# instaclustr/atsc

Hardware: AMD Instinct MI355X
Metric: Msamples/sec compressed (auto, e=5%) (higher is better)
Workload: dtype f64; 1 GPU; BASELINE.json configs[2] per GPU: 10,485,760 f64 samples, 40960 frames x 256, --compressor auto, e=5% (max_error=(float)5/100), classes C0-C4 cycled per 65536-sample block, inputs resident in HBM; the timed loop rotates over 5 different resident batches (series ids 0..4, batch b with the block -> class mapping shifted by 2 b); frames_per_gpu=40960, frame_len=256, encoded_bytes_rank0=3592754, parallelism=single GPU, GPU_MAX_HW_QUEUES=4

## Files before the change

atsc_amd/csrc/atsc_device.h:

```cpp
#pragma once
#include <hip/hip_runtime.h>
#include <stdint.h>

#include "../../include/atsc_hip.h"
#include "atsc_internal.h"

#include <map>
#include <mutex>
#include <utility>

namespace atsc {

#define DEVI __device__ __forceinline__
template <int W = 0>
DEVI uint32_t tid_now()
{
    uint32_t t = (W == 1) ? __builtin_amdgcn_mbcnt_hi(~0u, __builtin_amdgcn_mbcnt_lo(~0u, 0u)) : threadIdx.x;
    asm volatile("" : "+v"(t));
    return t;
}

inline hipError_t ensure_dyn_lds(const void *fn, uint32_t bytes)
{
    static std::mutex mu;
// ... 158 lines not shown
    v += dpp_u32<0x111, 0xf>(v);
    v += dpp_u32<0x112, 0xf>(v);
    v += dpp_u32<0x114, 0xf>(v);
    v += dpp_u32<0x118, 0xf>(v);
    v += dpp_u32<0x142, 0xa>(v);
    v += dpp_u32<0x143, 0xc>(v);
    return v;
}
DEVI uint32_t wave_max_u32(uint32_t v)
{
    v = max(v, dpp_u32<0xb1, 0xf>(v));
    v = max(v, dpp_u32<0x4e, 0xf>(v));
    v = max(v, dpp_u32<0x124, 0xf>(v));
    v = max(v, dpp_u32<0x128, 0xf>(v));
    v = max(v, dpp_u32<0x142, 0xa>(v));
    v = max(v, dpp_u32<0x143, 0xc>(v));
    return (uint32_t)__builtin_amdgcn_readlane((int)v, 63);
}
DEVI uint32_t wave_min_u32(uint32_t v) { return ~wave_max_u32(~v); }
template <int CTRL, int ROWMASK>
DEVI double dpp_f64(double v)
{
    const int lo = __builtin_amdgcn_update_dpp(0, __double2loint(v), CTRL, ROWMASK, 0xf, false);
    const int hi = __builtin_amdgcn_update_dpp(0, __double2hiint(v), CTRL, ROWMASK, 0xf, false);
    return __hiloint2double(hi, lo);
}
template <int CTRL>
DEVI double dpp_f64_full(double v)
{
    const int lo = __builtin_amdgcn_mov_dpp(__double2loint(v), CTRL, 0xf, 0xf, true);
    const int hi = __builtin_amdgcn_mov_dpp(__double2hiint(v), CTRL, 0xf, 0xf, true);
    return __hiloint2double(hi, lo);
}
DEVI double wave_sum_f64(double v)
{
    v += dpp_f64_full<0xb1>(v);
    v += dpp_f64_full<0x4e>(v);
    v += dpp_f64_full<0x124>(v);
    v += dpp_f64_full<0x128>(v);
    v += dpp_f64<0x142, 0xa>(v);
    v += dpp_f64<0x143, 0xc>(v);
    const int lo = __builtin_amdgcn_readlane(__double2loint(v), 63);
    const int hi = __builtin_amdgcn_readlane(__double2hiint(v), 63);
    return __hiloint2double(hi, lo);
}

template <int FN, int T, int MAXIT = 0, typename F>
DEVI void for_strided(uint32_t tid, uint32_t n, F &&f)
{
    if constexpr (FN != 0) {
#pragma unroll
        for (int m = 0; m < (FN + T - 1) / T; ++m) {
            const uint32_t j = tid + (uint32_t)(m * T);
            if (FN % T == 0 || j < (uint32_t)FN) f(j);
        }
    } else if constexpr (MAXIT != 0) {
#pragma unroll
        for (int m = 0; m < MAXIT; ++m) {
            const uint32_t j = tid + (uint32_t)(m * T);
            if (j < n) f(j);
        }
    } else {
        for (uint32_t j = tid; j < n; j += T) f(j);
    }
}

template <int W>
DEVI double block_sum_f64(double v, double *red, int &parity)
{
    v = wave_sum_f64(v);
    if (W == 1) return v;
    double *r = red + parity * 16;
    parity ^= 1;
    if ((tid_now<W>() & 63) == 0) r[tid_now<W>() >> 6] = v;
    __syncthreads();
    double s = r[0];
#pragma unroll
    for (int w = 1; w < W; ++w) s += r[w];
    return s;
}
template <int W>
DEVI uint32_t block_sum_u32(uint32_t v, double *red, int &parity)
{
    v = wave_sum_u32(v);
    if (W == 1) return v;
    uint32_t *r = (uint32_t *)(red + parity * 16);
    parity ^= 1;
    if ((tid_now<W>() & 63) == 0) r[tid_now<W>() >> 6] = v;
    __syncthreads();
    uint32_t s = r[0];
#pragma unroll
    for (int w = 1; w < W; ++w) s += r[w];
    return s;
}

template <int CTRL, int ROWMASK>
DEVI double dpp_f64_self(double v)
{
    const int lo = __builtin_amdgcn_update_dpp(__double2loint(v), __double2loint(v), CTRL, ROWMASK, 0xf, false);
    const int hi = __builtin_amdgcn_update_dpp(__double2hiint(v), __double2hiint(v), CTRL, ROWMASK, 0xf, false);
    return __hiloint2double(hi, lo);
}
template <bool IsMin>
DEVI double wave_minmax_f64(double v)
{
#define ATSC_MM_STEP(O)                                          \
    {                                                            \
        const double o = O;                                      \
        v = IsMin ? fmin(o, v) : fmax(o, v);                     \
    }
    ATSC_MM_STEP(dpp_f64_full<0xb1>(v))
    ATSC_MM_STEP(dpp_f64_full<0x4e>(v))
    ATSC_MM_STEP(dpp_f64_full<0x124>(v))
    ATSC_MM_STEP(dpp_f64_full<0x128>(v))
    ATSC_MM_STEP((dpp_f64_self<0x142, 0xa>(v)))
    ATSC_MM_STEP((dpp_f64_self<0x143, 0xc>(v)))
// ... 227 lines not shown
    return X;
}

template <typename KnotFn>
DEVI double spline_eval(KnotFn V, uint32_t i, uint32_t n, uint32_t step, uint32_t K, uint32_t magic)
{
    if (i == n - 1) return V(K - 1);
    uint32_t seg = (step == 1) ? i : __umulhi(i, magic);
    if (seg > K - 2) seg = K - 2;
    const uint32_t t0i = seg * step;
    const uint32_t t1i = (seg + 1 == K - 1) ? (n - 1) : (seg + 1) * step;
    const double t0 = (double)t0i, t1 = (double)t1i;
    const double v0 = V(seg), v1 = V(seg + 1);
    const double nt = ((double)i - t0) / (t1 - t0);
    if (seg > 0 && K - seg > 2) {
        const uint32_t tmi = (seg - 1) * step;
        const uint32_t tpi = (seg + 2 == K - 1) ? (n - 1) : (seg + 2) * step;
        const double tm = (double)tmi, tp = (double)tpi;
        const double vm = V(seg - 1), vp = V(seg + 2);
        const double t2 = nt * nt;
        const double t3 = t2 * nt;
        const double two_t3 = t3 * 2.0;
        const double two_t2 = t2 * 2.0;
        const double three_t2 = t2 * 3.0;
        const double m0 = (v1 - vm) / (t1 - tm) * (t1 - t0);
        const double m1 = (vp - v0) / (tp - t0) * (t1 - t0);
        return v0 * (two_t3 - three_t2 + 1.0) + m0 * (t3 - two_t2 + nt) + v1 * (three_t2 - two_t3) +
               m1 * (t3 - t2);
    }
    return v0 * (1.0 - nt) + v1 * nt;
}

DEVI double div1e5(double r)
{
    const double y = 1.0e-5;
    const double q = r * y;
    const double rem = fma(-q, 100000.0, r);
    return fma(rem, y, q);
}
DEVI bool wide_range(double mn, double mx) { return !(fabs(mn) < 1e150 && fabs(mx) < 1e150); }
DEVI double div1e5_fix(double r, double o, bool wide) { return (wide && isinf(r)) ? r : o; }

DEVI double recip_abs(double g)
{
    const double a = fabs(g);
    if (a > 1e-290 && a < 1e290) {
        double r = __builtin_amdgcn_rcp(a);
        r = fma(fma(-a, r, 1.0), r, r);
        r = fma(fma(-a, r, 1.0), r, r);
        return r;
    }
    return 1.0 / a;
}
DEVI double mape_term(double o, double g)
{
    const double a = fabs(g), d = fabs(o - g);
    return (a > 1e-290 && a < 1e290) ? d * recip_abs(g) : d / a;
}
DEVI bool tiny_range(double mn, double mx) { return !(mn > 1e-290 || mx < -1e-290); }
DEVI double spline_term_slow(double sv, double mn, double mx, double g)
{
    double o = round(sv * 100000.0) / 100000.0;
    if (o < mn) o = mn;
    else if (o > mx) o = mx;
    return fabs((o - g) / g);
}
DEVI double fft_term_slow(float v, double mn, double mx, double g)
{
    double o = round((double)v * 100000.0) / 100000.0;
    if (o > mx) o = mx;
    if (o < mn) o = mn;
    return fabs((o - g) / g);
}

DEVI float hp_norm(uint64_t e) { return __uint_as_float((uint32_t)(e >> 32)); }
DEVI void hp_sift_down_range(uint64_t *h, uint32_t pos, uint32_t end)
{
    const uint64_t elt = h[pos];
    const float en = hp_norm(elt);
    uint32_t child = 2 * pos + 1;
    while (end >= 2 && child <= end - 2) {
        const uint64_t c0 = h[child], c1 = h[child + 1];
        const bool right = !(hp_norm(c0) > hp_norm(c1));
        const uint64_t c = right ? c1 : c0;
        child += right ? 1u : 0u;
        if (en >= hp_norm(c)) { h[pos] = elt; return; }
        h[pos] = c;
        pos = child;
        child = 2 * pos + 1;
    }
    if (end >= 1 && child == end - 1) {
        const uint64_t c = h[child];
        if (!(en >= hp_norm(c))) { h[pos] = c; pos = child; }
    }
    h[pos] = elt;
}
DEVI void hp_rebuild(uint64_t *h, uint32_t len)
{
    for (uint32_t n = len / 2; n > 0;) {
        --n;
        hp_sift_down_range(h, n, len);
    }
}
DEVI void hp_rebuild_parallel(uint64_t *h, uint32_t len, uint32_t tid, uint32_t nthreads)
{
    if (len < 2) return;
// ... 235 lines not shown
```

atsc_amd/csrc/atsc_host.cpp:

```cpp
#include <hip/hip_runtime.h>

#include <algorithm>
#include <chrono>
#include <cmath>
#include <cstdio>
#include <cstdlib>
#include <cstring>
#include <limits>
#include <map>
#include <memory>
#include <mutex>
#include <new>
#include <thread>
#include <string>
#include <vector>

#include "atsc_host_private.h"

namespace atsc {
hipError_t launch_compress_class(int cls, uint32_t count, uint32_t lds, const double *samples,
                                 const DevFrame *frames, const uint32_t *ids, const DevPlan *plans,
                                 const float2 *twpool, const KParams &prm, uint8_t *slots,
                                 DevResult *res, atsc_frame_diag *diag, const UniArgs &uni, hipStream_t s,
                                 hipEvent_t ev0 = nullptr, hipEvent_t ev1 = nullptr);
// ... 612 lines not shown
        } else {
            pi = it->second;
        }
        const DevPlan &dp = p->tabs.plans[pi];
        const int c = class_of(n, dp.L);
        if (c < 0) { atsc_plan_destroy(p); return fail(ctx, ATSC_E_UNSUPPORTED, "plan_create: frame class"); }
        cls[f] = c;
        p->class_count[c]++;
        p->class_lds[c] = std::max(p->class_lds[c], dp.lds_bytes);
        if (c == CLASS_LARGE) p->ws_stride = std::max(p->ws_stride, large_ws_bytes(n, dp.L, dp.kcap));
        frames[f].sample_off = frame_off[f];
        frames[f].slot_off = slot;
        frames[f].n = n;
        frames[f].plan = pi;
        const uint64_t pb = atsc_payload_bound_bytes(n);
        slot += (pb + 15) & ~15ull;
        bound += pb + 16;
    }
    p->n_samples = frame_off[n_frames] - frame_off[0];
    p->h_frames = frames;
    p->slot_bytes = slot;
    p->body_bound = bound;
    std::vector<uint32_t> ids(n_frames);
    {
        uint32_t acc = 0;
        for (int c = 0; c < N_CLASSES; ++c) { p->class_first[c] = acc; acc += p->class_count[c]; }
        std::vector<uint32_t> cur(p->class_first);
        for (uint64_t f = 0; f < n_frames; ++f) ids[cur[cls[f]]++] = (uint32_t)f;
    }
    p->class_uni.assign(N_CLASSES, UniArgs());
    for (int c = 0; c < N_CLASSES; ++c) {
        UniArgs &u = p->class_uni[c];
        memset(&u, 0, sizeof(u));
        const uint32_t cnt = p->class_count[c];
        if (!cnt) continue;
        const uint32_t *cid = ids.data() + p->class_first[c];
        const DevFrame &f0 = frames[cid[0]];
        const uint64_t stride = (atsc_payload_bound_bytes(f0.n) + 15) & ~15ull;
        bool ok = true;
        for (uint32_t i = 0; i < cnt && ok; ++i) {
            const DevFrame &f = frames[cid[i]];
            ok = cid[i] == cid[0] + i && f.plan == f0.plan &&
                 f.sample_off == f0.sample_off + (uint64_t)i * f0.n &&
                 f.slot_off == f0.slot_off + (uint64_t)i * stride;
        }
        if (ok && c != CLASS_LARGE && !getenv("ATSC_NO_UNIFORM")) {
            u.enabled = 1;
            u.fid0 = cid[0];
            u.sample_off0 = f0.sample_off;
            u.slot_off0 = f0.slot_off;
            u.slot_stride = stride;
            u.n = f0.n;
            u.plan = f0.plan;
        }
    }
    p->large_tiled = choose_large_tiled(p->class_count[CLASS_LARGE]);
    if (p->class_count[CLASS_LARGE]) {
        std::vector<uint32_t> lp;
        for (uint64_t f = 0; f < n_frames; ++f)
            if (cls[f] == CLASS_LARGE) lp.push_back(frames[f].plan);
        std::sort(lp.begin(), lp.end());
        lp.erase(std::unique(lp.begin(), lp.end()), lp.end());
        p->large_pre = large_pre_extents(p->tabs.plans, lp);
        p->large_pre.even_off = 1;
        for (uint64_t f = 0; f < n_frames; ++f)
            if (cls[f] == CLASS_LARGE && (frames[f].sample_off & 1ull)) p->large_pre.even_off = 0;
    }
    int rc = upload_tables(ctx, p->tabs);
    if (rc) { atsc_plan_destroy(p); return rc; }
    const uint32_t nb = (uint32_t)((n_frames + 1023) / 1024);
#define PCHK(call)                                                                     \
    do {                                                                               \
        hipError_t e__ = (call);                                                       \
        if (e__ != hipSuccess) { atsc_plan_destroy(p); return fail(ctx, ATSC_E_HIP, #call, e__); } \
    } while (0)
    PCHK(pool_alloc(ctx, (void **)&p->d_frames, n_frames * sizeof(DevFrame)));
    PCHK(hipMemcpy(p->d_frames, frames.data(), n_frames * sizeof(DevFrame), hipMemcpyHostToDevice));
    PCHK(pool_alloc(ctx, (void **)&p->d_ids, n_frames * sizeof(uint32_t)));
    PCHK(hipMemcpy(p->d_ids, ids.data(), n_frames * sizeof(uint32_t), hipMemcpyHostToDevice));
    PCHK(pool_alloc(ctx, (void **)&p->d_res, n_frames * sizeof(DevResult)));
    p->slots_bytes = std::max<uint64_t>(slot, 16);
    PCHK(pool_alloc(ctx, (void **)&p->d_slots, p->slots_bytes));
    PCHK(pool_alloc(ctx, (void **)&p->d_local, n_frames * sizeof(uint32_t)));
    PCHK(pool_alloc(ctx, (void **)&p->d_blocksum, (nb + 1) * sizeof(uint64_t)));
    if (p->class_count[CLASS_LARGE]) {
        p->ws_slots = (std::min<uint32_t>(p->class_count[CLASS_LARGE], large_ws_slots(p->ws_stride)) + 3u) & ~3u;
        PCHK(pool_alloc(ctx, (void **)&p->d_ws, p->ws_stride * p->ws_slots));
    }
#undef PCHK
    *out = p;
    return ATSC_OK;
    ATSC_API_END
}
extern "C" uint64_t atsc_plan_n_frames(const atsc_plan *p) { return p ? p->n_frames : 0; }
extern "C" uint64_t atsc_plan_n_samples(const atsc_plan *p) { return p ? p->n_samples : 0; }
extern "C" uint64_t atsc_plan_body_bound(const atsc_plan *p) { return p ? p->body_bound : 0; }

static const uint32_t COMPRESSION_SPEED[7] = {0x7fffffffu, 4096, 2048, 1024, 512, 256, 128};

static int build_sub(atsc_ctx *ctx, const atsc_plan *plan, uint32_t min_n, uint32_t force_n, bool nopad,
                     bool want_res, SubPlan **out)
{
    *out = nullptr;
    SubPlan *t = new (std::nothrow) SubPlan();
    if (!t) return ATSC_E_NOMEM;
    t->min_n = min_n;
// ... 312 lines not shown
            int rc = build_sub(ctx, plan, 0, 0, true, false, &t);
            if (rc) return rc;
            plan->nopad = t;
        }
        int rc = launch_sub(ctx, plan, plan->nopad, d_samples, prm, S.d_slots, S.d_res, d_diag, s, ws_set);
        if (rc) return rc;
        return pack();
    }
    int dominant = 0, last_c = 0;
    if (adapt) { prm.cost = CH.d_cost; want_order = true; }
    for (int c = 1; c < N_CLASSES; ++c)
        if (plan->class_count[c] > plan->class_count[dominant]) dominant = c;
    for (int c = 0; c < N_CLASSES; ++c)
        if (plan->class_count[c]) last_c = c;
    for (int c = 0; c < N_CLASSES; ++c) {
        if (!plan->class_count[c]) continue;
        const bool timed = ctx->profiling && c == dominant;
        const bool bracket = timed && c == CLASS_LARGE;
        hipEvent_t ev0 = nullptr, ev1 = nullptr;
        if (timed) {
            if (ctx->ev_used == ctx->ev_pool.size()) {
                hipEvent_t a, b;
                HIPCHK(ctx, hipEventCreateWithFlags(&a, hipEventReleaseToDevice));
                HIPCHK(ctx, hipEventCreateWithFlags(&b, hipEventReleaseToDevice));
                ctx->ev_pool.emplace_back(a, b);
            }
            ev0 = ctx->ev_pool[ctx->ev_used].first;
            ev1 = ctx->ev_pool[ctx->ev_used].second;
            if (bracket) HIPCHK(ctx, hipEventRecord(ev0, s));
        }
        if (pipelined && c == last_c && c != CLASS_LARGE && !ev1) {
            ev1 = CH.ev_codec;
            codec_attached = true;
        }
        hipError_t e;
        if (c == CLASS_LARGE) {
            KParams lp = prm;
            lp.large_tiled = plan->large_tiled ? 1u : 0u;
            const bool pre = plan->large_pre.tiles1 && (compressor == ATSC_AUTO || compressor == ATSC_FFT);
            e = launch_compress_large(plan->class_count[c], d_samples, plan->d_frames, plan->d_ids + plan->class_first[c],
                                      plan->tabs.d_plans, plan->tabs.d_tw, lp, S.d_slots, S.d_res, d_diag, ws_set,
                                      plan->ws_stride, plan->ws_slots, s, pre ? &plan->large_pre : nullptr);
        }
        else {
            UniArgs u = plan->class_uni[c];
            u.adaptive = (ids_main != plan->d_ids) ? 1u : 0u;
            u.count = plan->class_count[c];
            u.spread = 0;
            if (u.enabled && !u.adaptive && u.count >= 4096) {
                uint32_t sp = (uint32_t)((double)u.count * 0.6180339887) | 1u;
                auto gcd = [](uint32_t a, uint32_t b) { while (b) { const uint32_t t = a % b; a = b; b = t; } return a; };
                while (gcd(sp, u.count) != 1) sp += 2;
                u.spread = sp % u.count;
            }
            e = launch_compress_class(c, plan->class_count[c], plan->class_lds[c], d_samples,
                                      plan->d_frames, ids_main + plan->class_first[c],
                                      plan->tabs.d_plans, plan->tabs.d_tw, prm, S.d_slots,
                                      S.d_res, d_diag, u, s, ev0, ev1);
        }
        if (e != hipSuccess) return fail(ctx, ATSC_E_HIP, "launch k_compress", e);
        if (bracket) HIPCHK(ctx, hipEventRecord(ev1, s));
        if (timed) ctx->ev_used++;
    }
    return pack();
}

extern "C" int atsc_compress_plan_dev(atsc_ctx *ctx, const atsc_plan *plan, const double *d_samples,
                                      int compressor, int bounded, float max_error, int sample_level,
                                      uint8_t *d_body, uint64_t body_cap, uint64_t *d_rec_off,
                                      uint8_t *d_chosen, double *d_err, void *stream)
{
    ATSC_API_BEGIN
    return compress_impl(ctx, plan, d_samples, compressor, bounded, max_error, sample_level, d_body,
                         body_cap, d_rec_off, d_chosen, d_err, stream, false);
    ATSC_API_END
}
extern "C" int atsc_compress_plan_dev_pipelined(atsc_ctx *ctx, const atsc_plan *plan,
                                                const double *d_samples, int compressor, int bounded,
                                                float max_error, int sample_level, uint8_t *d_body,
                                                uint64_t body_cap, uint64_t *d_rec_off,
                                                uint8_t *d_chosen, double *d_err, void *stream)
{
    ATSC_API_BEGIN
    return compress_impl(ctx, plan, d_samples, compressor, bounded, max_error, sample_level, d_body,
                         body_cap, d_rec_off, d_chosen, d_err, stream, true);
    ATSC_API_END
}
extern "C" int atsc_ctx_set_adaptive_order(atsc_ctx *ctx, int on)
{
    if (!ctx) return ATSC_E_INVALID;
    ctx->adaptive_order = on != 0;
    return ATSC_OK;
}
extern "C" int atsc_plan_join(atsc_ctx *ctx, const atsc_plan *plan, void *stream)
{
    if (!ctx || !plan) return fail(ctx, ATSC_E_INVALID, "plan_join: null argument");
    for (int i = 0; i < 8; ++i)
        if (plan->chains[i].pending) HIPCHK(ctx, hipStreamWaitEvent((hipStream_t)stream, plan->chains[i].ev_done, 0));
    return ATSC_OK;
}
extern "C" int atsc_plan_input_release(atsc_ctx *ctx, const atsc_plan *plan, void *stream)
{
    if (!ctx || !plan) return fail(ctx, ATSC_E_INVALID, "plan_input_release: null argument");
    for (int i = 0; i < 8; ++i)
        if (plan->chains[i].pending) HIPCHK(ctx, hipStreamWaitEvent((hipStream_t)stream, plan->chains[i].ev_codec, 0));
    return ATSC_OK;
// ... 849 lines not shown
```

atsc_amd/csrc/atsc_internal.h:

```cpp
#pragma once
#include <stdint.h>
#include <new>
#include <stdexcept>
#include <vector>

namespace atsc {

struct DevPlan {
    uint32_t n;
    uint32_t L;
    uint32_t pre;
    uint32_t bins;
    uint32_t mf;
    uint32_t dk1;
    uint32_t dk2;
    uint32_t kcap;
    uint32_t direct;
    uint32_t half;
    uint32_t M;
    uint32_t sc;
    uint32_t nstages;
    uint32_t radix[14];
    uint32_t stmagic[14];
    uint32_t p2bins;
// ... 46 lines not shown
    uint64_t slot_off;
    uint32_t n;
    uint32_t plan;
};

struct DevResult {
    double err;
    uint32_t len;
    uint32_t chosen;
};

struct KParams {
    double max_err;
    double poly_target;
    double poly_q_hi;
    double poly_q_lo;
    int32_t max_err_m;
    int32_t mode;
    int32_t bounded;
    int32_t want_diag;
    int32_t debug_stop;
    int32_t trial;
    uint32_t trial_min_n;
    const DevResult *trial_res;
    uint32_t *cost;
    uint32_t large_tiled;
    uint32_t sparse_inv;
    uint32_t prestats;
    uint32_t tile_stats;
    uint32_t fast_skip;
    uint32_t prefft;
};
struct LargePre {
    uint32_t tiles1, tiles2, chunks;
    uint32_t m1_max, m2_max;
    uint32_t sp_tiles;
    uint32_t chunks_n;
    uint32_t cols243;
    uint32_t rows9p;
    uint32_t even_off;
};
constexpr uint32_t LARGE_SPLIT_MAX = 128;

struct UniArgs {
    uint32_t enabled;
    uint32_t adaptive;
    uint32_t fid0;
    uint64_t sample_off0;
    uint64_t slot_off0;
    uint64_t slot_stride;
    uint32_t n;
    uint32_t plan;
    uint32_t spread, count;
};

struct DevDFrame {
    uint64_t payload_off;
    uint64_t out_off;
    uint32_t payload_len;
    uint32_t n;
    uint32_t tag;
    uint32_t plan;
};

struct DevWTask {
    uint64_t dst;
    uint32_t frame;
    uint32_t lo, hi;
    uint32_t pad;
};
struct DevWGather {
    uint64_t src, dst;
    uint32_t len, pad;
};

constexpr uint32_t AGG_TILE = 2048;
struct DevAggPart {
    double sum, mn, mx;
    uint64_t count;
};
enum : uint32_t { AGG_FIRST = 1, AGG_LAST = 2 };
struct DevAggTile {
    uint64_t src, dst;
    uint32_t lo, hi;
    uint32_t win, flags;
};
struct DevAggComb {
    uint64_t head, tail, mid, dst;
    uint32_t n, g, win, final_;
};

struct DevMomPart {
    double mx, m2x, mt, m2t, c;
    uint64_t n;
};
struct DevPosTile {
    uint64_t src, dst, t0;
    uint32_t lo, hi;
};

struct DevDltPart {
    double up, down, after_falls, max_rise, max_fall;
    uint64_t pairs, rises, falls;
};
enum : uint32_t { DLT_CONT = 1, DLT_CARRY = 2 };
struct DevDltTile {
    uint64_t src, dst;
// ... 146 lines not shown
```

atsc_amd/csrc/atsc_kernels.hip:

```cpp
#include <hip/hip_runtime.h>
#include <hip/hip_ext.h>
#include <stdint.h>
#include <stdlib.h>
#include <algorithm>
#include <string.h>

#include "atsc_device.h"

namespace atsc {

template <int W>
DEVI void fft_untangle(const DevPlan &P, const float2 *Z, float2 *out, const float2 *tw)
{
    constexpr int T = 64 * W;
    const uint32_t M = P.M;
    for (uint32_t k = tid_now<W>(); k <= M; k += T) {
        const float2 zk = Z[k == M ? 0 : k];
        const float2 zm = Z[k == 0 ? 0 : M - k];
        const float2 a = make_float2(zk.x + zm.x, zk.y - zm.y);
        const float2 b = make_float2(zk.x - zm.x, zk.y + zm.y);
        const float2 t = cmul_conj_tw(make_float2(b.y, -b.x), tw[k]);
        out[k] = make_float2(0.5f * a.x + 0.5f * t.x, 0.5f * a.y + 0.5f * t.y);
    }
    __syncthreads();
// ... 210 lines not shown
        const uint32_t ra = rec[i];
        const uint64_t ka = (uint64_t)__double_as_longlong(xs[ra & 0xffffu]);
        uint32_t r = 0;
        for (uint32_t j = q; j < count; j += p) {
            const uint32_t rb = rec[j];
            const uint64_t kb = (uint64_t)__double_as_longlong(xs[rb & 0xffffu]);
            r += (kb < ka || (kb == ka && rb < ra)) ? 1u : 0u;
        }
        if (p == 1) rank[i] = r;
        else if (r) atomicAdd(&rank[i], r);
    }
    __syncthreads();
    for (uint32_t i = tid; i < count; i += T) tmp[rank[i]] = rec[i];
    __syncthreads();
    for (uint32_t i = tid; i < count; i += T) rec[i] = tmp[i];
    __syncthreads();
}

#ifdef ATSC_STAMPS
__device__ unsigned long long g_phase_cyc[64 * 16];
__device__ unsigned long long g_frame_span[4 * 65536 * 3];
#define PH(i) do { if (FN != 0) { const long long now_ = clock64(); \
    if (tid == 0) atomicAdd(&ph_acc[i], (unsigned long long)(now_ - ph_t)); ph_t = clock64(); } } while (0)
#else
#define PH(i) do {} while (0)
#endif
template <int W, int SPL, bool IDW, int FN, bool LEAN_ = (FN != 0)>
__device__ __forceinline__ void compress_frame(
    const double *__restrict__ samples, const DevFrame *__restrict__ frames,
    const uint32_t *__restrict__ ids, const DevPlan *__restrict__ plans,
    const float2 *__restrict__ twpool, const KParams &prm, uint8_t *__restrict__ slots,
    DevResult *__restrict__ res, atsc_frame_diag *__restrict__ diag, const UniArgs &uni, const uint32_t bid)
{
    constexpr int T = 64 * W;
    constexpr bool FIX_ = FN != 0;
    extern __shared__ __attribute__((aligned(16))) unsigned char smem[];
    const uint32_t tid = tid_now<W>();
    uint32_t fid;
    DevFrame fr;
    const long long t_start = prm.cost ? clock64() : 0;
#ifdef ATSC_STAMPS
    __shared__ unsigned long long ph_acc[16];
    if (tid < 16) ph_acc[tid] = 0;
    __syncthreads();
    long long ph_t = clock64();
    const uint32_t span0 = 3u * 65536u * (((uint32_t)prm.debug_stop >> 24) & 3u);
    if (FN != 0 && tid == 0 && bid < 65536) {
        g_frame_span[span0 + 3 * bid] = wall_clock64();
        g_frame_span[span0 + 3 * bid + 2] = (unsigned long long)__builtin_amdgcn_s_getreg((31 << 11) | (0 << 6) | 4) |
                                           ((unsigned long long)__builtin_amdgcn_s_getreg((31 << 11) | (0 << 6) | 20) << 32);
    }
#endif
    if (FIX_ || uni.enabled) {
        const uint32_t r = uni.adaptive ? (uint32_t)__builtin_amdgcn_readfirstlane((int)(ids[bid] - uni.fid0))
                           : uni.spread ? (uint32_t)(((uint64_t)bid * uni.spread) % uni.count) : bid;
        fid = uni.fid0 + r;
        fr.sample_off = uni.sample_off0 + (uint64_t)r * uni.n;
        fr.slot_off = uni.slot_off0 + (uint64_t)r * uni.slot_stride;
        fr.n = uni.n;
        fr.plan = uni.plan;
    } else {
        fid = ids[bid];
        fr = frames[fid];
    }
    typedef const __attribute__((address_space(4))) DevPlan PlanConst;
    PlanConst &P = *(PlanConst *)(plans + fr.plan);
#define P_GENERIC (*(const DevPlan *)&P)
    constexpr bool FIX = FN != 0;
    constexpr bool LEAN = LEAN_;
    static_assert(LEAN || !FIX, "fixed-length instantiations are lean");
    constexpr uint32_t cL = FIX ? cx_next_size(FIX ? FN : 1) : 0, cmf = (3 >= FN / 100) ? 3 : FN / 100;
    static_assert(!FIX || (FN >= 128 && cL <= 64 * W * SPL), "fixed-length instantiation");
    constexpr bool chalf = cL % 2 == 0;
    constexpr uint32_t cM = chalf ? cL / 2 : cL;
    const uint32_t n = FIX ? FN : P.n, L = FIX ? cL : P.L, pre = FIX ? (cL - FN) / 2 : P.pre;
    const uint32_t bins = FIX ? cL / 2 + 1 : P.bins;
    const uint32_t mf = FIX ? cmf : P.mf;
    constexpr uint32_t cdk1 = cmf / 2 > 1 ? cmf / 2 : 1, cdk2 = cmf / 10 > 1 ? cmf / 10 : 1;
    constexpr uint32_t ckcap = (cL / 2 + 1 < cmf + 17 * cdk1 + 5 * cdk2) ? cL / 2 + 1 : cmf + 17 * cdk1 + 5 * cdk2;
    const uint32_t dk1 = FIX ? cdk1 : P.dk1, dk2 = FIX ? cdk2 : P.dk2;
    constexpr EncLds lay = enc_lds(FIX ? FN : 1, FIX ? cL : 1, FIX ? cM : 1, false, ckcap, W == 1);
    const uint32_t o_xs = FIX ? lay.o_xs : P.o_xs, o_tw = FIX ? lay.o_tw : P.o_tw, o_ab = FIX ? lay.o_ab : P.o_ab;
    const uint32_t ab_half = FIX ? lay.ab_half : P.ab_half, ab_bytes = FIX ? lay.ab_bytes : P.ab_bytes;
    const uint32_t o_sel = FIX ? lay.o_sel : P.o_sel, o_aux = FIX ? lay.o_aux : P.o_aux, o_red = FIX ? lay.o_red : P.o_red;
    const uint32_t o_hist = FIX ? lay.o_hist : P.o_hist;
    const uint32_t kcap = FIX ? ckcap : P.kcap;

    double *xs = (double *)(smem + o_xs);
    float2 *tw = (float2 *)(smem + o_tw);
    unsigned char *AB = smem + o_ab;
    float2 *A = (float2 *)AB;
    float2 *B = (float2 *)(AB + ab_half);
    Sel *sel = (Sel *)(smem + o_sel);
    uint32_t *aux = (uint32_t *)(smem + o_aux);
    double *red = (double *)(smem + o_red);
    uint32_t *wsum = (W == 1) ? (uint32_t *)red : (uint32_t *)(red + 32);
    int parity = 0;

    uint8_t *out = slots + fr.slot_off;
    int mode = LEAN ? (int)ATSC_AUTO : prm.mode;
    const bool bounded = LEAN ? true : (prm.bounded != 0);

    constexpr bool REGSTAT = FIX && W == 1 && (FN == 256 || FN == 512);
    bool reg_stats = false;
    double rs_mn = 0.0, rs_mx = 0.0;
    uint32_t rs_frac = 0, rs_pk = 0;
    {
        const double *src = samples + fr.sample_off;
        if constexpr (REGSTAT) {
            if ((fr.sample_off & 1ull) == 0) {
                constexpr int NP = FN / 128;
                const double2 *src2 = (const double2 *)src;
                double2 *xs2 = (double2 *)xs;
                double2 v[NP];
#pragma unroll
                for (int m = 0; m < NP; ++m) v[m] = src2[tid + 64 * m];
#pragma unroll
                for (int m = 0; m < NP; ++m) xs2[tid + 64 * m] = v[m];
                const double x0 = lane_f64(v[0].x, 0);
                rs_mn = x0;
                rs_mx = x0;
#pragma unroll
                for (int m = 0; m < NP; ++m) {
                    const double a = v[m].x, b = v[m].y;
                    rs_frac |= (frac_nonzero(a) || frac_nonzero(b)) ? 1u : 0u;
                    if (a > rs_mx) rs_mx = a;
                    if (a < rs_mn) rs_mn = a;
                    if (b > rs_mx) rs_mx = b;
                    if (b < rs_mn) rs_mn = b;
                    double left = wave_shr1_f64(b);
                    if (m > 0) {
                        const double wrap = lane_f64(v[m - 1].y, 63);
                        left = (tid == 0) ? wrap : left;
                    }
                    const uint32_t jx = 2u * (tid + 64u * (uint32_t)m);
                    if (jx == 0 || a != left) rs_pk += (vlen(jx) << 13) | 1u;
                    if (b != a) rs_pk += (vlen(jx + 1) << 13) | 1u;
                }
                reg_stats = true;
            }
        }
        if (reg_stats) {
        } else if (((fr.sample_off | n) & 1ull) == 0) {
            const double2 *src2 = (const double2 *)src;
            double2 *xs2 = (double2 *)xs;
            for_strided<FN / 2, T, (SPL + 1) / 2>(tid, n >> 1, [&](uint32_t j) { xs2[j] = src2[j]; });
        } else {
            for (uint32_t j = tid; j < n; j += T) xs[j] = src[j];
        }
    }
    __syncthreads();

    PH(0);
    double smin, smax;
    uint32_t bitdepth;
    uint32_t stat_pk = 0;
    bool stat_pk_done = false;
    {
        double mn, mx;
        uint32_t fr_any = 0;
        if (reg_stats) {
            mn = rs_mn; mx = rs_mx; fr_any = rs_frac;
        } else {
            const double x0 = xs[0];
            mn = x0; mx = x0;
            for_strided<FN, T, SPL>(tid, n, [&](uint32_t j) {
                const double v = xs[j];
                fr_any |= frac_nonzero(v) ? 1u : 0u;
                if (v > mx) mx = v;
                if (v < mn) mn = v;
                if constexpr (W > 1) {
                    const double b = xs[j ? j - 1 : 0];
                    if (j == 0 || v != b) stat_pk += (vlen(j) << 13) | 1u;
                }
            });
        }
        if constexpr (W > 1) {
            const BlockStats bs = block_stats4<W>(mn, mx, fr_any, stat_pk, red, wsum);
            mn = bs.mn; mx = bs.mx; fr_any = bs.frac; stat_pk = bs.pk;
            stat_pk_done = true;
        } else {
            mn = block_minmax_f64<W, true>(mn, red, parity);
            mx = block_minmax_f64<W, false>(mx, red, parity);
            fr_any = block_or_u32<W>(fr_any, red, parity);
        }
        smin = mn;
        smax = mx;
        if (mn == 0.0 || mx == 0.0) {
            uint32_t mni = 0xFFFFFFFFu, mxi = 0xFFFFFFFFu;
            for_strided<FN, T, SPL>(tid, n, [&](uint32_t j) {
                const double v = xs[j];
                if (v == mn) mni = min(mni, j);
                if (v == mx) mxi = min(mxi, j);
            });
            mni = block_min_u32<W>(mni, red, parity);
            mxi = block_min_u32<W>(mxi, red, parity);
            if (mni < n) smin = xs[mni];
            if (mxi < n) smax = xs[mxi];
        }
        int64_t maxi, mini;
        bool fz;
        split_n(smax, maxi, fz);
// ... 52 lines not shown

    if (!LEAN && prm.debug_stop == 2) return;
    double g[SPL], inv[SPL];

    if (!LEAN && prm.debug_stop == 3) return;
    const bool run_fft = (mode == ATSC_AUTO || mode == ATSC_FFT);
    const bool run_poly = (mode == ATSC_AUTO || mode == ATSC_POLYNOMIAL || mode == ATSC_IDW);
    const bool run_rle = (mode == ATSC_AUTO || mode == ATSC_RLE);
    const bool idw = IDW && (mode == ATSC_IDW);
    const double me = prm.max_err;
    const bool prune = LEAN ? true : (mode == ATSC_AUTO) && (0.0 <= me);
    uint32_t best_size = 0xFFFFFFFFu;
    int best_owner = 3;
    auto can_win = [&](uint32_t size_lb, int owner) {
        return size_lb < best_size || (size_lb == best_size && owner < best_owner);
    };
    auto offer = [&](uint32_t size, int owner) {
        if (can_win(size, owner)) { best_size = size; best_owner = owner; }
    };
    uint32_t fft_k = 0, fft_size = 0xFFFFFFFFu, fft_trips = 0;
    double fft_err = 0.0;
    bool fft_done = false;
    const float mxf = (float)smax, mnf = (float)smin;
    uint32_t poly_step = 1, poly_K = 0, poly_size = 0xFFFFFFFFu, poly_trips = 0;
    double poly_err = 0.0;
    bool poly_done = false;
    uint32_t psz_step = 0, psz_K = 0xFFFFFFFFu, psz = 0;
    auto poly_payload_size = [&](uint32_t step, uint32_t K) -> uint32_t {
        if (step == psz_step && K == psz_K) return psz;
        uint32_t vb = 0;
        if (bitdepth == 0 || bitdepth == 3) {
            vb = K * (bitdepth == 0 ? 8u : 1u);
        } else {
            for (uint32_t k = tid; k < K; k += T) {
                const uint32_t t = (k == K - 1) ? (n - 1) : k * step;
                vb += value_bytes(bitdepth, xs[t]);
            }
            vb = block_sum_u32<W>(vb, red, parity);
        }
        psz_step = step;
        psz_K = K;
        psz = 1 + 1 + vlen(K) + vb + 8 + 8 + 1;
        return psz;
    };

    uint32_t rle_size = 0xFFFFFFFFu, rle_R = 0, rle_D = 0, rle_ib = 0, rle_lb = 0xFFFFFFFFu;
    bool rle_sorted = false, rle_pending = false;
    bool rle_early = false;
    uint32_t *rrec_std = (uint32_t *)AB;
    uint32_t *rhp_std = rrec_std + n;
    uint32_t *rph_std = (uint32_t *)tw;
    auto run_key = [&](uint32_t rec) { return (uint64_t)__double_as_longlong(xs[rec & 0xffffu]); };
    auto rle_sort_and_group = [&](uint32_t *rrec, uint32_t *rhp, uint32_t *rph) {
        __syncthreads();
        for (uint32_t j = tid; j < n; j += T)
            aux[j] = (j + 1 >= n || xs[j + 1] != xs[j]) ? 1u : 0u;
        __syncthreads();
        const uint32_t R = block_excl_scan<W>(aux, n, wsum);
        uint32_t *ends = rhp;
        for (uint32_t j = tid; j < n; j += T)
            if (j + 1 >= n || xs[j + 1] != xs[j]) ends[aux[j]] = j;
        __syncthreads();
        for (uint32_t r = tid; r < R; r += T) {
            const uint32_t st = r ? ends[r - 1] + 1 : 0;
            rrec[r] = (st << 16) | ends[r];
        }
        __syncthreads();
        if (R <= 512 && 2 * R <= n + 2) {
            block_rank_sort_runs<W>(rrec, xs, R, aux);
        } else {
            uint32_t p2 = 1;
            while (p2 < R) p2 <<= 1;
            block_sort_runs<W>(rrec, xs, R, p2);
        }
        for (uint32_t i = tid; i < R; i += T)
            aux[i] = (i == 0 || run_key(rrec[i]) != run_key(rrec[i - 1])) ? 1u : 0u;
        __syncthreads();
        const uint32_t D = block_excl_scan<W>(aux, R, wsum);
        for (uint32_t i = tid; i < R; i += T)
            if (i == 0 || run_key(rrec[i]) != run_key(rrec[i - 1])) rhp[aux[i]] = i;
        if (tid == 0) rhp[D] = R;
        __syncthreads();
        uint32_t hb = 0;
        for (uint32_t gi = tid; gi < D; gi += T) {
            const uint32_t h0 = rhp[gi], h1 = rhp[gi + 1];
            const uint32_t b = value_bytes(bitdepth, xs[rrec[h0] & 0xffffu]) + vlen(h1 - h0);
            rph[gi] = b;
            hb += b;
        }
        __syncthreads();
        hb = block_sum_u32<W>(hb, red, parity);
        rle_R = R;
        rle_D = D;
        rle_size = 2 + vlen(D) + hb + rle_ib;
        rle_sorted = true;
    };
    bool rle_small = false;
    struct RleLane { uint32_t rec, cnt, hb, D, hb_total; bool head, live; };
    auto rle_small_build = [&]() {
        uint32_t *srt = (uint32_t *)AB, *ends = srt + 16;
        __syncthreads();
        const uint32_t C = (n + 63) >> 6, j0 = tid * C;
        uint32_t cnt = 0;
        for (uint32_t k = 0; k < C; ++k) {
            const uint32_t j = j0 + k;
            if (j < n && (j + 1 >= n || xs[j + 1] != xs[j])) ++cnt;
// ... 38 lines not shown
        const uint32_t next = after ? tid + 1 + (uint32_t)__builtin_ctzll(after) : R;
        g.cnt = next - tid;
        g.hb = g.head ? value_bytes(bitdepth, xs[g.rec & 0xffffu]) + vlen(g.cnt) : 0u;
        g.hb_total = wave_sum_u32(g.hb);
        return g;
    };
    if (run_rle) {
        uint32_t pk = 0;
        if (stat_pk_done) {
            pk = stat_pk;
        } else {
            if (reg_stats) {
                pk = rs_pk;
            } else {
                for_strided<FN, T, SPL>(tid, n, [&](uint32_t j) {
                    const double a = xs[j], b = xs[j ? j - 1 : 0];
                    if (j == 0 || a != b) pk += (vlen(j) << 13) | 1u;
                });
            }
            pk = block_sum_u32<W>(pk, red, parity);
        }
        rle_R = pk & 0x1fffu;
        rle_ib = pk >> 13;
        const uint32_t minval = (bitdepth == 0) ? 8u : 1u;
        rle_lb = 3 + rle_ib + (rle_R >= 2 ? 2u : 1u) * (minval + 1);
        if (W == 1 && rle_R <= 16 && ab_bytes >= 128) {
            rle_small_build();
            const RleLane g = rle_small_group();
            rle_D = g.D;
            rle_size = 2 + vlen(g.D) + g.hb_total + rle_ib;
            rle_small = true;
            rle_early = true;
            if (prune) offer(rle_size, 2);
        } else if (mode == ATSC_RLE) {
            rle_sort_and_group(rrec_std, rhp_std, rph_std);
            rle_sorted = true;
        } else if (rle_R <= 64 && 12 * rle_R + 16 <= ab_bytes) {
            uint32_t *e_rec = (uint32_t *)AB;
            rle_sort_and_group(e_rec, e_rec + rle_R, e_rec + 2 * rle_R + 1);
            rle_sorted = false;
            rle_early = true;
            if (prune) offer(rle_size, 2);
        } else {
            rle_pending = true;
        }
    }

    PH(2);
    if (!LEAN && prm.debug_stop == 10) return;
    if (!(prune && best_size < 19)) {
#pragma unroll
        for (int m = 0; m < SPL; ++m) {
            const uint32_t j = tid + m * T;
            if (j < L) {
                int32_t i = (int32_t)j - (int32_t)pre;
                i = i < 0 ? 0 : (i >= (int32_t)n ? (int32_t)n - 1 : i);
                g[m] = xs[i];
                inv[m] = recip_abs(g[m]);
            } else {
                g[m] = 1.0;
                inv[m] = 0.0;
            }
        }
    }

    PH(3);
    if (!LEAN && prm.debug_stop == 11) return;
    bool poly_first = false;
    if (prune && run_fft && run_poly && smax != smin) {
        poly_first = poly_payload_size(P.pstep[0], P.pK[0]) < 1 + 1 + 9 * min(mf, bins) + 8;
    }
    constexpr bool POLY2GO = W >= 16;
    double poly_cur = prm.max_err + 1.0;
    bool poly_paused = false;
    auto eval_poly = [&](const bool first_go) {
        if (run_poly) {
            bool poly_pruned = false;
            if (smax == smin) {
                poly_K = 0;
                poly_step = 1;
            } else if (!bounded) {
                poly_step = P.pstep[0];
                poly_K = P.pK[0];
            } else {
                double2 *mm = (double2 *)AB;
                const double inv_n = P.inv_n;
                const bool pfast = !wide_range(smin, smax) && !has_sub;
                const bool nozero = smin > 0.0 || smax < 0.0;
                double cur = POLY2GO ? poly_cur : prm.max_err + 1.0;
                while (round(cur * 10000.0) > prm.poly_q_hi) {
                    const uint32_t ti = poly_trips;
                    const uint32_t step = P.pstep[ti];
                    const uint32_t K = P.pK[ti];
                    if (prune && !can_win(poly_payload_size(step, K), 1)) { poly_pruned = true; break; }
                    ++poly_trips;
                    poly_step = step;
                    poly_K = K;
                    const bool same_trip = ti > 0 && step == P.pstep[ti - 1] && K == P.pK[ti - 1];
                    if (same_trip) {
                    } else if (IDW && step > 1 && idw) {
                        double s = 0.0;
#pragma unroll
                        for (int m = 0; m < SPL; ++m) {
                            const uint32_t j = tid + m * T;
                            if (j >= pre && j < pre + n) {
                                const double x = (double)(j - pre);
                                double num = 0.0, den = 0.0, hitv = 0.0;
                                bool hit = false;
                                for (uint32_t k = 0; k < K; ++k) {
                                    const uint32_t pk = (k == K - 1) ? (n - 1) : k * step;
                                    const double v = xs[pk];
                                    const double d = fabs((double)pk - x);
                                    if (d == 0.0) {
                                        if (!hit) { hit = true; hitv = v; }
                                    } else if (!hit) {
                                        const double w = 1.0 / (d * d);
// ... 92 lines not shown
                            double o = div1e5(round(sv * 100000.0));
                            o = fmin(fmax(o, smin), smax);
                            return fabs(o - g[m]) * inv[m];
                        };
                        double t1 = 0.0;
                        bool fails = false;
                        if (SPL >= 2 && pfast && nozero) {
                            t1 = term(1);
                            const double lb = block_sum_f64<W>(t1, red, parity) * inv_n;
                            if (round(lb * 10000.0) > prm.poly_q_hi) { cur = lb; fails = true; }
                        }
                        if (!fails) {
                            double s = 0.0;
#pragma unroll
                            for (int m = 0; m < SPL; ++m) s += (m == 1 && SPL >= 2 && pfast && nozero) ? t1 : term(m);
                            s = block_sum_f64<W>(s, red, parity);
                            cur = s * inv_n;
                        }
                    }
                    if (poly_trips > 22) {
                        if (round(cur * 10000.0) < prm.poly_q_lo) break;
                        poly_step = 1; poly_K = n; cur = 0.0;
                        break;
                    }
                    if (K == n) { cur = 0.0; break; }
                    if (POLY2GO && first_go && round(cur * 10000.0) > prm.poly_q_hi) {
                        poly_cur = cur;
                        poly_paused = true;
                        return;
                    }
                }
                poly_err = cur;
            }
            poly_size = poly_payload_size(poly_step, poly_K);
            poly_done = !poly_pruned;
            if (prune && poly_done && poly_err <= me) offer(poly_size, 1);
            dg.poly_size = poly_size; dg.poly_trips = (uint16_t)poly_trips;
            dg.poly_step = (uint16_t)poly_step; dg.poly_points = poly_K; dg.poly_err = poly_err;
        }

    };

    if (poly_first) eval_poly(true);
    PH(4);
    if (!LEAN && prm.debug_stop == 13) return;
    if (run_fft) {
        if (mxf == mnf) {
            fft_k = 0;
            fft_size = 1 + 1 + 8;
            fft_done = true;
        } else if (prune && !can_win(1 + 1 + 9 + 8, 0)) {
        } else {
            rle_early = false;
            {
                const float2 *twp = twpool + P.tw_off;
                for_strided<FIX ? (int)cL : 0, T, SPL>(tid, L, [&](uint32_t j) { tw[j] = twp[j]; });
            }
            float2 *spec;
            if (FIX && chalf) {
                float *Af = (float *)A;
#pragma unroll
                for (int m = 0; m < SPL; ++m) {
                    const uint32_t j = tid + m * T;
                    if (j < L) Af[j] = (float)g[m];
                }
                __syncthreads();
                float2 *Z = fft_forward_fixed<W, FIX ? cM : 2, 2>(A, B, tw);
                spec = (Z == A) ? B : A;
                fft_untangle_fixed<W, FIX ? cM : 2>(Z, spec, tw);
            } else if (FIX) {
#pragma unroll
                for (int m = 0; m < SPL; ++m) {
                    const uint32_t j = tid + m * T;
                    if (j < L) A[j] = make_float2((float)g[m], 0.0f);
                }
                __syncthreads();
                spec = fft_forward_fixed<W, FIX ? cM : 3, 1>(A, B, tw);
            } else if (P.direct) {
                __syncthreads();
                dft_direct<W>(P_GENERIC, xs, A, tw);
                spec = A;
            } else if (P.half) {
                float *Af = (float *)A;
#pragma unroll
                for (int m = 0; m < SPL; ++m) {
                    const uint32_t j = tid + m * T;
                    if (j < L) Af[j] = (float)g[m];
                }
                __syncthreads();
                float2 *Z = fft_forward<W>(P_GENERIC, A, B, tw);
                spec = (Z == A) ? B : A;
                fft_untangle<W>(P_GENERIC, Z, spec, tw);
            } else {
#pragma unroll
                for (int m = 0; m < SPL; ++m) {
                    const uint32_t j = tid + m * T;
                    if (j < L) A[j] = make_float2((float)g[m], 0.0f);
                }
                __syncthreads();
                spec = fft_forward<W>(P_GENERIC, A, B, tw);
            }
            PH(5);
            if (!LEAN && prm.debug_stop == 4) return;
            constexpr int KPL = (SPL * 32 + 1 + 63) / 64;
            uint32_t nb[KPL];
            float bre[KPL], bim[KPL];
            uint64_t *keys = (uint64_t *)(spec == A ? B : A);
            bool heap_order = false;
            uint32_t hlen = 0;
            uint32_t sorted_n = 0;
            uint32_t nz = 0;
            if (W == 1) {
#pragma unroll
                for (int m = 0; m < KPL; ++m) {
                    const uint32_t k = tid + 64 * m;
                    nb[m] = 0;
                    bre[m] = 0.0f;
                    bim[m] = 0.0f;
                    if (k < bins) {
                        const float2 z = spec[k];
                        bre[m] = z.x;
                        bim[m] = z.y;
                        nb[m] = __float_as_uint(
                            (float)sqrt((double)z.x * (double)z.x + (double)z.y * (double)z.y));
                        nz += (z.x != 0.0f || z.y != 0.0f) ? 1u : 0u;
                    }
                }
            } else {
                for (uint32_t k = tid; k < bins; k += T) {
                    const float2 z = spec[k];
                    const float nrm = (float)sqrt((double)z.x * (double)z.x + (double)z.y * (double)z.y);
                    keys[k] = ((uint64_t)(~__float_as_uint(nrm)) << 32) | (uint64_t)k;
                    nz += (z.x != 0.0f || z.y != 0.0f) ? 1u : 0u;
                }
                __syncthreads();
            }
            const uint32_t Z = block_sum_u32<W>(nz, red, parity);
            bool keys_fresh = true;
            auto build_order = [&](const uint32_t want) {
                if (!keys_fresh) {
                    __syncthreads();
                    for (uint32_t k = tid; k < bins; k += T) {
                        const float2 z = spec[k];
                        const float nrm = (float)sqrt((double)z.x * (double)z.x + (double)z.y * (double)z.y);
                        keys[k] = ((uint64_t)(~__float_as_uint(nrm)) << 32) | (uint64_t)k;
                    }
                    __syncthreads();
                }
                keys_fresh = false;
                uint32_t nk = bins;
                if (bins > want && want > 0) {
                    uint32_t *hist = (uint32_t *)(smem + o_hist);
                    const uint32_t few = 2 * want + 16;
                    uint64_t prefix = 0, resolved = 0;
                    uint32_t remaining = want;
                    for (int shift = 56; shift >= 0; shift -= 8) {
                        if (shift == 24 || shift == 16) continue;
                        for (uint32_t i = tid; i < 256; i += T) hist[i] = 0;
                        __syncthreads();
                        for (uint32_t k = tid; k < bins; k += T) {
                            const uint64_t v = keys[k];
                            if ((v & resolved) == prefix) atomicAdd(&hist[(uint32_t)(v >> shift) & 255u], 1u);
                        }
                        __syncthreads();
                        if (tid < 64) {
                            const uint32_t c0 = hist[4 * tid], c1 = hist[4 * tid + 1], c2 = hist[4 * tid + 2], c3 = hist[4 * tid + 3];
                            const uint32_t sum = c0 + c1 + c2 + c3;
                            const uint32_t incl = wave_incl_scan_u32(sum);
                            const uint64_t reach = __ballot(incl >= remaining);
                            if (reach && tid == (uint32_t)__builtin_ctzll(reach)) {
                                uint32_t cum = incl - sum, d = 4 * tid, in = c0;
                                if (cum + c0 < remaining) { cum += c0; ++d; in = c1;
// ... 108 lines not shown
                            const uint32_t pos = (uint32_t)(keys[heap_order ? bins - 1 - i : i] & 0xffffffffu);
                            const float2 z = spec[pos];
                            sel[i].pos = pos; sel[i].re = z.x; sel[i].im = z.y;
                            const double cf = ((pos == 0 || 2 * pos == L) ? 1.0 : 2.0) * invL;
                            Stg e;
                            e.pos = pos;
                            e.stp = mod_magic(pos * (uint32_t)T, L, magicL);
                            e.a = (float)(cf * (double)z.x);
                            e.b = (float)(cf * (double)z.y);
                            stg[tid] = e;
                        }
                        __syncthreads();
#pragma unroll 2
                        for (uint32_t i = 0; i < cnt; ++i) {
                            const Stg e = stg[i];
                            const bool isdc = e.pos == 0;
                            dc = isdc ? e.a : dc;
                            const float a = isdc ? 0.0f : e.a, b = isdc ? 0.0f : e.b;
                            uint32_t idx = mod_magic(e.pos * tid, L, magicL);
#pragma unroll
                            for (int m = 0; m < SPL; ++m) {
                                const float2 w = tw[idx];
                                acc[m] = fmaf(a, w.x, acc[m]);
                                acc[m] = fmaf(-b, w.y, acc[m]);
                                idx += e.stp;
                                idx = min(idx, idx - L);
                            }
                        }
                        used += cnt;
                    }
                }
                for (; used < K; ++used) {
                    uint32_t pos;
                    float2 z;
                    if (W == 1) {
                        pos = 0;
                        if (!heap_order) {
                            uint32_t lm = nb[0];
#pragma unroll
                            for (int m = 1; m < KPL; ++m) lm = max(lm, nb[m]);
                            const uint32_t wm = wave_max_u32(lm);
                            uint32_t mult = 0;
#pragma unroll
                            for (int m = KPL - 1; m >= 0; --m) {
                                const uint64_t bal = __ballot(nb[m] == wm);
                                mult += (uint32_t)__popcll(bal);
                                if (bal) pos = 64u * (uint32_t)m + (uint32_t)__builtin_ctzll(bal);
                            }
                            if (mult > 1) {
                                __syncthreads();
#pragma unroll
                                for (int m = 0; m < KPL; ++m) {
                                    const uint32_t k = tid + 64 * m;
                                    if (k < bins) {
                                        const float nrm = (float)sqrt((double)bre[m] * (double)bre[m] +
                                                                      (double)bim[m] * (double)bim[m]);
                                        keys[k] = ((uint64_t)__float_as_uint(nrm) << 32) | (uint64_t)k;
                                    }
                                }
                                __syncthreads();
                                hp_rebuild_parallel(keys, bins, tid, 64u);
                                hlen = bins;
                                for (uint32_t i = 0; i < used; ++i) (void)hp_pop(keys, hlen);
                                heap_order = true;
                            }
                        }
                        if (heap_order) pos = (uint32_t)(hp_pop(keys, hlen) & 0xffffffffu);
                        float zr = 0.0f, zi = 0.0f;
#pragma unroll
                        for (int m = 0; m < KPL; ++m) {
                            if (tid + 64 * m == pos) nb[m] = 0;
                            if ((pos >> 6) == (uint32_t)m) { zr = bre[m]; zi = bim[m]; }
                        }
                        z = make_float2(__uint_as_float(__builtin_amdgcn_readlane(__float_as_uint(zr), pos & 63)),
                                        __uint_as_float(__builtin_amdgcn_readlane(__float_as_uint(zi), pos & 63)));
                    } else {
                        pos = (uint32_t)(keys[heap_order ? bins - 1 - used : used] & 0xffffffffu);
                        z = spec[pos];
                    }
                    if (tid == 0) { sel[used].pos = pos; sel[used].re = z.x; sel[used].im = z.y; }
                    big += (pos >= 251) ? 1u : 0u;
                    const double cf = ((pos == 0 || 2 * pos == L) ? 1.0 : 2.0) * invL;
                    const float a = (float)(cf * (double)z.x);
                    const float b = (float)(cf * (double)z.y);
                    if (pos == 0) {
                        dc = a;
                    } else {
                        uint32_t idx = mod_magic(pos * tid, L, magicL);
                        const uint32_t stp = mod_magic(pos * (uint32_t)T, L, magicL);
#pragma unroll
                        for (int m = 0; m < SPL; ++m) {
                            const float2 w = tw[idx];
                            acc[m] = fmaf(a, w.x, acc[m]);
                            acc[m] = fmaf(-b, w.y, acc[m]);
                            idx += stp;
                            idx = min(idx, idx - L);
                        }
                    }
                }
                PH(7);
                if (!bounded) { cur = 0.0; break; }
                double s = 0.0;
                if (__builtin_expect(fast_clamp, 1)) {
#pragma unroll
                    for (int m = 0; m < SPL; ++m) {
                        const double x5 = (double)(acc[m] + dc) * 100000.0;
                        double o = div1e5(trunc(x5 + copysign(0.5, x5)));
// ... 707 lines not shown
```

Before: 102,500 Msamples/s.

## Prefetch FFT twiddles early, vectorize twiddle copy, batch reciprocals, cheapen spread modulo

```diff
diff --git a/atsc_amd/csrc/atsc_device.h b/atsc_amd/csrc/atsc_device.h
--- a/atsc_amd/csrc/atsc_device.h
+++ b/atsc_amd/csrc/atsc_device.h
@@ -234,7 +234,7 @@
 #pragma unroll
         for (int m = 0; m < (FN + T - 1) / T; ++m) {
             const uint32_t j = tid + (uint32_t)(m * T);
-            if (FN % T == 0 || j < (uint32_t)FN) f(j);
+            if ((m + 1) * T <= FN || j < (uint32_t)FN) f(j);
         }
     } else if constexpr (MAXIT != 0) {
 #pragma unroll
@@ -244,6 +244,31 @@
         }
     } else {
         for (uint32_t j = tid; j < n; j += T) f(j);
+    }
+}
+template <int CB, int T>
+DEVI bool slice_in(int m, uint32_t j, uint32_t bound)
+{
+    return (CB != 0 && (m + 1) * T <= CB) || j < bound;
+}
+template <int CN, int T, int NS, typename V>
+DEVI void walk_load(V (&r)[NS], const V *__restrict__ src, uint32_t tid, uint32_t cnt)
+{
+#pragma unroll
+    for (int m = 0; m < NS; ++m) {
+        if (CN != 0 && m * T >= CN) continue;
+        const uint32_t j = tid + (uint32_t)(m * T);
+        r[m] = src[(CN != 0 && (m + 1) * T <= CN) ? j : min(j, cnt - 1u)];
+    }
+}
+template <int CN, int T, int NS, typename V>
+DEVI void walk_store(const V (&r)[NS], V *dst, uint32_t tid, uint32_t cnt)
+{
+#pragma unroll
+    for (int m = 0; m < NS; ++m) {
+        if (CN != 0 && m * T >= CN) continue;
+        const uint32_t j = tid + (uint32_t)(m * T);
+        if (slice_in<CN, T>(m, j, cnt)) dst[j] = r[m];
     }
 }
 
@@ -577,6 +602,28 @@
     }
     return 1.0 / a;
 }
+template <int N>
+DEVI void recip_abs_all(const double (&g)[N], double (&inv)[N])
+{
+    bool any_out = false;
+#pragma unroll
+    for (int m = 0; m < N; ++m) {
+        const double a = fabs(g[m]);
+        double r = __builtin_amdgcn_rcp(a);
+        r = fma(fma(-a, r, 1.0), r, r);
+        r = fma(fma(-a, r, 1.0), r, r);
+        inv[m] = r;
+        any_out |= !(a > 1e-290 && a < 1e290);
+    }
+    if (__ballot(any_out)) {
+#pragma unroll
+        for (int m = 0; m < N; ++m) {
+            const double a = fabs(g[m]);
+            const double q = 1.0 / a;
+            inv[m] = (a > 1e-290 && a < 1e290) ? inv[m] : q;
+        }
+    }
+}
 DEVI double mape_term(double o, double g)
 {
     const double a = fabs(g), d = fabs(o - g);
diff --git a/atsc_amd/csrc/atsc_host.cpp b/atsc_amd/csrc/atsc_host.cpp
--- a/atsc_amd/csrc/atsc_host.cpp
+++ b/atsc_amd/csrc/atsc_host.cpp
@@ -688,6 +688,7 @@
             u.slot_stride = stride;
             u.n = f0.n;
             u.plan = f0.plan;
+            u.tw_off = p->tabs.plans[f0.plan].tw_off;
         }
     }
     p->large_tiled = choose_large_tiled(p->class_count[CLASS_LARGE]);
@@ -1106,6 +1107,7 @@
                 auto gcd = [](uint32_t a, uint32_t b) { while (b) { const uint32_t t = a % b; a = b; b = t; } return a; };
                 while (gcd(sp, u.count) != 1) sp += 2;
                 u.spread = sp % u.count;
+                u.spread_m = spread_magic(u.count);
             }
             e = launch_compress_class(c, plan->class_count[c], plan->class_lds[c], d_samples,
                                       plan->d_frames, ids_main + plan->class_first[c],
diff --git a/atsc_amd/csrc/atsc_internal.h b/atsc_amd/csrc/atsc_internal.h
--- a/atsc_amd/csrc/atsc_internal.h
+++ b/atsc_amd/csrc/atsc_internal.h
@@ -122,7 +122,16 @@
     uint32_t n;
     uint32_t plan;
     uint32_t spread, count;
-};
+    uint64_t spread_m;
+    uint64_t tw_off;
+};
+ATSC_HD constexpr uint64_t spread_magic(uint32_t d) { return d > 1 ? ~0ull / d + 1ull : 0ull; }
+ATSC_HD constexpr uint32_t spread_mod(uint32_t x, uint64_t m, uint32_t d)
+{
+    const uint64_t frac = m * x;
+    const uint64_t lo = (frac & 0xffffffffull) * d, hi = (frac >> 32) * d + (lo >> 32);
+    return (uint32_t)(hi >> 32);
+}
 
 struct DevDFrame {
     uint64_t payload_off;
diff --git a/atsc_amd/csrc/atsc_kernels.hip b/atsc_amd/csrc/atsc_kernels.hip
--- a/atsc_amd/csrc/atsc_kernels.hip
+++ b/atsc_amd/csrc/atsc_kernels.hip
@@ -286,8 +286,11 @@
     }
 #endif
     if (FIX_ || uni.enabled) {
+        const uint64_t dealt = (uint64_t)bid * uni.spread;
         const uint32_t r = uni.adaptive ? (uint32_t)__builtin_amdgcn_readfirstlane((int)(ids[bid] - uni.fid0))
-                           : uni.spread ? (uint32_t)(((uint64_t)bid * uni.spread) % uni.count) : bid;
+                           : !uni.spread ? bid
+                           : (dealt >> 32) == 0 ? spread_mod((uint32_t)dealt, uni.spread_m, uni.count)
+                                                : (uint32_t)(dealt % uni.count);
         fid = uni.fid0 + r;
         fr.sample_off = uni.sample_off0 + (uint64_t)r * uni.n;
         fr.slot_off = uni.slot_off0 + (uint64_t)r * uni.slot_stride;
@@ -339,6 +342,28 @@
     bool reg_stats = false;
     double rs_mn = 0.0, rs_mx = 0.0;
     uint32_t rs_frac = 0, rs_pk = 0;
+    constexpr int TW4 = (SPL + 1) / 2;
+    typedef float f32x4 __attribute__((ext_vector_type(4)));
+    auto tw_copy = [&](const float2 *twp, const bool off_even) {
+        if ((L & 1u) == 0 && off_even) {
+            f32x4 r[TW4];
+            walk_load<FIX ? (int)cL / 2 : 0, T, TW4>(r, (const f32x4 *)twp, tid, L >> 1);
+            walk_store<FIX ? (int)cL / 2 : 0, T, TW4>(r, (f32x4 *)tw, tid, L >> 1);
+        } else {
+            float2 r[SPL];
+            walk_load<FIX ? (int)cL : 0, T, SPL>(r, twp, tid, L);
+            walk_store<FIX ? (int)cL : 0, T, SPL>(r, tw, tid, L);
+        }
+    };
+    constexpr bool TWPRE = FIX && W == 1 && cL % 2 == 0 && FN != 128;
+    bool tw_ready = false;
+    f32x4 twr[TW4];
+    if constexpr (TWPRE) {
+        tw_ready = (uni.tw_off & 1ull) == 0;
+        if (tw_ready) walk_load<(int)cL / 2, T, TW4>(twr, (const f32x4 *)(twpool + uni.tw_off), tid, cL / 2);
+    }
+#define TW_PUT() do { if constexpr (TWPRE) { \
+        if (tw_ready) walk_store<(int)cL / 2, T, TW4>(twr, (f32x4 *)tw, tid, cL / 2); } } while (0)
     {
         const double *src = samples + fr.sample_off;
         if constexpr (REGSTAT) {
@@ -349,6 +374,7 @@
                 double2 v[NP];
 #pragma unroll
                 for (int m = 0; m < NP; ++m) v[m] = src2[tid + 64 * m];
+                TW_PUT();
 #pragma unroll
                 for (int m = 0; m < NP; ++m) xs2[tid + 64 * m] = v[m];
                 const double x0 = lane_f64(v[0].x, 0);
@@ -382,6 +408,7 @@
         } else {
             for (uint32_t j = tid; j < n; j += T) xs[j] = src[j];
         }
+        if (!reg_stats) TW_PUT();
     }
     __syncthreads();
 
@@ -540,6 +567,7 @@
     uint32_t *rph_std = (uint32_t *)tw;
     auto run_key = [&](uint32_t rec) { return (uint64_t)__double_as_longlong(xs[rec & 0xffffu]); };
     auto rle_sort_and_group = [&](uint32_t *rrec, uint32_t *rhp, uint32_t *rph) {
+        tw_ready = false;
         __syncthreads();
         for (uint32_t j = tid; j < n; j += T)
             aux[j] = (j + 1 >= n || xs[j + 1] != xs[j]) ? 1u : 0u;
@@ -684,16 +712,15 @@
 #pragma unroll
         for (int m = 0; m < SPL; ++m) {
             const uint32_t j = tid + m * T;
-            if (j < L) {
-                int32_t i = (int32_t)j - (int32_t)pre;
-                i = i < 0 ? 0 : (i >= (int32_t)n ? (int32_t)n - 1 : i);
-                g[m] = xs[i];
-                inv[m] = recip_abs(g[m]);
-            } else {
-                g[m] = 1.0;
-                inv[m] = 0.0;
-            }
-        }
+            int32_t i = (int32_t)j - (int32_t)pre;
+            i = i < 0 ? 0 : (i >= (int32_t)n ? (int32_t)n - 1 : i);
+            const double x = xs[i];
+            g[m] = slice_in<FIX ? (int)cL : 0, T>(m, j, L) ? x : 1.0;
+        }
+        recip_abs_all<SPL>(g, inv);
+#pragma unroll
+        for (int m = 0; m < SPL; ++m)
+            if (!slice_in<FIX ? (int)cL : 0, T>(m, tid + m * T, L)) inv[m] = 0.0;
     }
 
     PH(3);
@@ -892,9 +919,9 @@
         } else if (prune && !can_win(1 + 1 + 9 + 8, 0)) {
         } else {
             rle_early = false;
-            {
-                const float2 *twp = twpool + P.tw_off;
-                for_strided<FIX ? (int)cL : 0, T, SPL>(tid, L, [&](uint32_t j) { tw[j] = twp[j]; });
+            if (!tw_ready) {
+                const uint64_t tw_off = P.tw_off;
+                tw_copy(twpool + tw_off, (tw_off & 1ull) == 0);
             }
             float2 *spec;
             if (FIX && chalf) {
@@ -902,7 +929,7 @@
 #pragma unroll
                 for (int m = 0; m < SPL; ++m) {
                     const uint32_t j = tid + m * T;
-                    if (j < L) Af[j] = (float)g[m];
+                    if (slice_in<FIX ? (int)cL : 0, T>(m, j, L)) Af[j] = (float)g[m];
                 }
                 __syncthreads();
                 float2 *Z = fft_forward_fixed<W, FIX ? cM : 2, 2>(A, B, tw);
@@ -912,7 +939,7 @@
 #pragma unroll
                 for (int m = 0; m < SPL; ++m) {
                     const uint32_t j = tid + m * T;
-                    if (j < L) A[j] = make_float2((float)g[m], 0.0f);
+                    if (slice_in<FIX ? (int)cL : 0, T>(m, j, L)) A[j] = make_float2((float)g[m], 0.0f);
                 }
                 __syncthreads();
                 spec = fft_forward_fixed<W, FIX ? cM : 3, 1>(A, B, tw);
@@ -925,7 +952,7 @@
 #pragma unroll
                 for (int m = 0; m < SPL; ++m) {
                     const uint32_t j = tid + m * T;
-                    if (j < L) Af[j] = (float)g[m];
+                    if (slice_in<FIX ? (int)cL : 0, T>(m, j, L)) Af[j] = (float)g[m];
                 }
                 __syncthreads();
                 float2 *Z = fft_forward<W>(P_GENERIC, A, B, tw);
@@ -935,7 +962,7 @@
 #pragma unroll
                 for (int m = 0; m < SPL; ++m) {
                     const uint32_t j = tid + m * T;
-                    if (j < L) A[j] = make_float2((float)g[m], 0.0f);
+                    if (slice_in<FIX ? (int)cL : 0, T>(m, j, L)) A[j] = make_float2((float)g[m], 0.0f);
                 }
                 __syncthreads();
                 spec = fft_forward<W>(P_GENERIC, A, B, tw);
@@ -957,7 +984,7 @@
                     nb[m] = 0;
                     bre[m] = 0.0f;
                     bim[m] = 0.0f;
-                    if (k < bins) {
+                    if (slice_in<FIX ? (int)cL / 2 + 1 : 0, 64>(m, k, bins)) {
                         const float2 z = spec[k];
                         bre[m] = z.x;
                         bim[m] = z.y;
@@ -1172,7 +1199,7 @@
 #pragma unroll
                                 for (int m = 0; m < KPL; ++m) {
                                     const uint32_t k = tid + 64 * m;
-                                    if (k < bins) {
+                                    if (slice_in<FIX ? (int)cL / 2 + 1 : 0, 64>(m, k, bins)) {
                                         const float nrm = (float)sqrt((double)bre[m] * (double)bre[m] +
                                                                       (double)bim[m] * (double)bim[m]);
                                         keys[k] = ((uint64_t)__float_as_uint(nrm) << 32) | (uint64_t)k;
```

Result: faster. 107,300 Msamples/s, median of 6 (+4.7%).
